# FFTAI/Wiki-GRx-Gym

Measured on AMD Instinct MI355X. Metric: env-steps/sec GR1T1 rough-terrain @4096 envs, higher is better.
Workload: dtype f32

## Files before the change

wiki-grx-gym_amd/csrc/grx_ppo.hip:

```cpp
#include <hip/hip_runtime.h>
#include <stdint.h>
#include "../../include/grx_ppo.h"

namespace {
constexpr int MAXA = 32;
constexpr int NTHR = 256;
constexpr int NRED = 3 + MAXA;

__device__ inline float nmax(float a, float b) { return (a > b || a != a) ? a : b; }
__device__ inline float nmin(float a, float b) { return (a < b || a != a) ? a : b; }

__device__ inline double wave_sum(double v) {
#pragma unroll
    for (int o = 32; o > 0; o >>= 1) v += __shfl_down(v, o);
    return v;
}

template <int A>
__global__ __launch_bounds__(NTHR) void ppo_loss_kernel(int B, const float* __restrict__ mu, const float* __restrict__ stdp,
                                                         const float* __restrict__ value, const float* __restrict__ actions,
                                                         const float* __restrict__ old_logp, const float* __restrict__ old_mu,
                                                         const float* __restrict__ old_sigma, const float* __restrict__ adv_,
                                                         const float* __restrict__ ret_, const float* __restrict__ tv_,
                                                         float clip, float vcoef, int use_clipped,
                                                         float* __restrict__ d_mu, float* __restrict__ d_value, double* __restrict__ partials) {
    const int i = blockIdx.x * NTHR + threadIdx.x;
    float red[3 + A];
#pragma unroll
    for (int k = 0; k < 3 + A; ++k) red[k] = 0.f;
    if (i < B) {
        const float invB = 1.0f / (float)B;
        float sg[A], df[A];
        float logp = 0.f, kl = 0.f;
#pragma unroll
        for (int k = 0; k < A; ++k) {
            const float s = stdp[k], m = mu[(size_t)i * A + k];
            sg[k] = s;
            df[k] = actions[(size_t)i * A + k] - m;
            logp += -(df[k] * df[k]) / (2.0f * s * s) - logf(s) - 0.9189385332046727f;
            const float os = old_sigma[(size_t)i * A + k], dm = old_mu[(size_t)i * A + k] - m;
            kl += logf(s / os + 1.e-5f) + (os * os + dm * dm) / (2.0f * s * s) - 0.5f;
        }
        const float adv = adv_[i];
        const float ratio = expf(logp - old_logp[i]);
        const float lo = 1.0f - clip, hi = 1.0f + clip;
        const float rc = nmin(nmax(ratio, lo), hi);
        const float s1 = -adv * ratio, s2 = -adv * rc;
        const float surr = nmax(s1, s2);
        const float w1 = s1 > s2 ? 1.f : (s1 == s2 ? 0.5f : 0.f), w2 = 1.f - w1;
        const float in_range = (ratio >= lo && ratio <= hi) ? 1.f : 0.f;
        const float g_ratio = -adv * (w1 + w2 * in_range);
        const float g_logp = g_ratio * ratio * invB;
#pragma unroll
        for (int k = 0; k < A; ++k) {
            const float s = sg[k], inv2 = 1.0f / (s * s);
            const float half = 0.5f * inv2;
            const float np = 0.f * (g_logp * (((df[k] * df[k] * half) * half) * 2.0f * (2.0f * s)) - g_logp / s);
            d_mu[(size_t)i * A + k] = g_logp * df[k] * inv2 + np;
            red[3 + k] = g_logp * (df[k] * df[k] * inv2 / s - 1.0f / s) + np;
        }
        const float v = value[i], ret = ret_[i];
        float vl, gv;
        if (use_clipped) {
            const float tv = tv_[i];
            const float dv = v - tv;
            const float vc = tv + nmin(nmax(dv, -clip), clip);
            const float l1 = (v - ret) * (v - ret), l2 = (vc - ret) * (vc - ret);
            vl = nmax(l1, l2);
            const float u1 = l1 > l2 ? 1.f : (l1 == l2 ? 0.5f : 0.f), u2 = 1.f - u1;
            const float vin = (dv >= -clip && dv <= clip) ? 1.f : 0.f;
            gv = u1 * 2.0f * (v - ret) + (vin != 0.f ? u2 * 2.0f * (vc - ret) : 0.f);
        } else {
            vl = (ret - v) * (ret - v);
            gv = -2.0f * (ret - v);
        }
        d_value[i] = vcoef * gv * invB;
        red[0] = surr; red[1] = vl; red[2] = kl;
    }
    __shared__ double s_red[NTHR / 64][3 + A];
    const int lane = threadIdx.x & 63, wv = threadIdx.x >> 6;
#pragma unroll
    for (int k = 0; k < 3 + A; ++k) {
        const double t = wave_sum((double)red[k]);
        if (lane == 0) s_red[wv][k] = t;
    }
    __syncthreads();
    if (threadIdx.x < 3 + A) {
        double t = 0.0;
#pragma unroll
        for (int w = 0; w < NTHR / 64; ++w) t += s_red[w][threadIdx.x];
        partials[(size_t)blockIdx.x * NRED + threadIdx.x] = t;
    }
}

__global__ __launch_bounds__(64) void ppo_loss_finalize(int B, int A, int nblk, const double* __restrict__ partials,
                                                         const float* __restrict__ stdp, float vcoef, float ecoef,
                                                         float* __restrict__ out, float* __restrict__ d_std) {
    const int k = threadIdx.x;
    double t = 0.0;
    constexpr int STAGE = 4096;
    __shared__ double s_p[STAGE];
    const bool staged = nblk * NRED <= STAGE;
    if (staged) {
        for (int i = k; i < nblk * NRED; i += 64) s_p[i] = partials[i];
        __syncthreads();
    }
    if (k < 3 + A)
        for (int b = 0; b < nblk; ++b) t += staged ? s_p[b * NRED + k] : partials[(size_t)b * NRED + k];
    __shared__ double s_t[64];
    s_t[k] = t;
    __syncthreads();
    if (k >= 3 && k < 3 + A) d_std[k - 3] = (float)t - ecoef / stdp[k - 3];
    if (k == 0) {
        const float surr = (float)(s_t[0] / (double)B), vl = (float)(s_t[1] / (double)B), klm = (float)(s_t[2] / (double)B);
        float ent = 0.f;
        for (int a = 0; a < A; ++a) ent += 1.4189385332046727f + logf(stdp[a]);
        out[0] = surr; out[1] = vl; out[2] = surr + vcoef * vl - ecoef * ent; out[3] = klm;
    }
}

template <int A>
void launch(int nblk, hipStream_t st, int B, const float* mu, const float* stdp, const float* value, const float* actions,
            const float* old_logp, const float* old_mu, const float* old_sigma, const float* adv, const float* ret, const float* tv,
            float clip, float vcoef, int use_clipped, float* d_mu, float* d_value, double* partials) {
    hipLaunchKernelGGL(ppo_loss_kernel<A>, dim3(nblk), dim3(NTHR), 0, st, B, mu, stdp, value, actions, old_logp, old_mu, old_sigma,
                       adv, ret, tv, clip, vcoef, use_clipped, d_mu, d_value, partials);
}

constexpr int CS_ROWS = 256;
__global__ __launch_bounds__(256) void colsum_partial(int rows, int cols, const float* __restrict__ x, float* __restrict__ partials) {
    const int lane = threadIdx.x & 63, wv = threadIdx.x >> 6;
    const int col = blockIdx.x * 64 + lane;
    const int r0 = blockIdx.y * CS_ROWS, r1 = min(rows, r0 + CS_ROWS);
    float acc = 0.f;
    if (col < cols) {
        float a0 = 0.f, a1 = 0.f, a2 = 0.f, a3 = 0.f;
        int r = r0 + wv;
        for (; r + 12 < r1; r += 16) {
            a0 += x[(size_t)r * cols + col]; a1 += x[(size_t)(r + 4) * cols + col];
            a2 += x[(size_t)(r + 8) * cols + col]; a3 += x[(size_t)(r + 12) * cols + col];
        }
// ... 403 lines not shown
```

wiki-grx-gym_amd/rl/fused_loss.py:

```python
import ctypes as C
import os

import torch

_LIB = None


def load_ppo_library():
    global _LIB
    if _LIB is None:
        path = os.environ.get("GRX_PPO_LIB") or os.path.join(os.path.dirname(os.path.dirname(os.path.abspath(__file__))), "csrc", "libgrx_ppo.so")
        if not os.path.exists(path):
            raise RuntimeError(f"{path} is missing: build it with `python -c 'import __graft_entry__ as g; g.build()'` "
                               "(there is no silent fallback for CUDA tensors; set GRX_PPO_FUSED_LOSS=0 to use the torch expression)")
        lib = C.CDLL(path)
        fp = C.c_void_p
        lib.grx_ppo_loss.restype = C.c_int
        lib.grx_ppo_loss.argtypes = [C.c_int, C.c_int] + [fp] * 10 + [C.c_float, C.c_float, C.c_float, C.c_int] + [fp] * 5 + [C.c_void_p]
        lib.grx_ppo_loss_partials_size.restype = C.c_int
        lib.grx_ppo_loss_partials_size.argtypes = [C.c_int]
        lib.grx_ppo_colsum.restype = C.c_int
        lib.grx_ppo_colsum.argtypes = [C.c_int, C.c_int, fp, fp, fp, C.c_void_p]
        lib.grx_ppo_colsum_partials_size.restype = C.c_int
        lib.grx_ppo_colsum_partials_size.argtypes = [C.c_int, C.c_int]
# ... 63 lines not shown
        lib.grx_est_forward.argtypes = [fp, C.c_int, C.c_int, fp, C.c_int, fp, C.POINTER(C.c_int), fp, fp, C.c_void_p]
        lib.grx_gae_partials_size.restype = C.c_int
        lib.grx_gae_partials_size.argtypes = [C.c_int, C.c_int]
        lib.grx_gae_returns.restype = C.c_int
        lib.grx_gae_returns.argtypes = [C.c_int, C.c_int] + [fp] * 4 + [C.c_float] * 3 + [fp] * 10 + [C.c_void_p]
        lib.grx_gp_seed.restype = C.c_int
        lib.grx_gp_seed.argtypes = [C.c_int, C.c_int] + [fp] * 4 + [C.c_void_p]
        lib.grx_gp_gate.restype = C.c_int
        lib.grx_gp_gate.argtypes = [C.c_int, C.c_int] + [fp] * 3 + [C.c_void_p]
        lib.grx_gp_sqnorm_partials_size.restype = C.c_int
        lib.grx_gp_sqnorm_partials_size.argtypes = [C.c_int, C.c_int]
        lib.grx_gp_sqnorm.restype = C.c_int
        lib.grx_gp_sqnorm.argtypes = [C.c_int, C.c_int] + [fp] * 3 + [C.c_void_p]
        lib.grx_gp_gate_backward.restype = C.c_int
        lib.grx_gp_gate_backward.argtypes = [C.c_int, C.c_int] + [fp] * 8 + [C.c_void_p]
        lib.grx_gp_seed_backward.restype = C.c_int
        lib.grx_gp_seed_backward.argtypes = [C.c_int, C.c_int] + [fp] * 8 + [C.c_void_p]
        lib.grx_ln_elu_forward.restype = C.c_int
        lib.grx_ln_elu_forward.argtypes = [C.c_int, C.c_int, fp, fp, fp, C.c_float, fp, fp, fp, C.c_void_p]
        lib.grx_ln_elu_backward_partials_size.restype = C.c_int
        lib.grx_ln_elu_backward_partials_size.argtypes = [C.c_int, C.c_int]
        lib.grx_ln_elu_backward.restype = C.c_int
        lib.grx_ln_elu_backward.argtypes = [C.c_int, C.c_int] + [fp] * 11 + [C.c_void_p]
        _LIB = lib
    return _LIB


TAIL_MAX = 24


class _TailTensors(C.Structure):
    _fields_ = [("n", C.c_int), ("pad", C.c_int), ("param", C.c_void_p * TAIL_MAX), ("grad", C.c_void_p * TAIL_MAX),
                ("exp_avg", C.c_void_p * TAIL_MAX), ("exp_avg_sq", C.c_void_p * TAIL_MAX), ("step", C.c_void_p * TAIL_MAX),
                ("numel", C.c_longlong * TAIL_MAX)]


class _TailArgs(C.Structure):
    _fields_ = [("loss", C.c_void_p), ("bad_flag", C.c_void_p), ("kl", C.c_void_p), ("lr", C.c_void_p), ("value_loss", C.c_void_p),
                ("surrogate_loss", C.c_void_p), ("sums", C.c_void_p), ("partials", C.c_void_p), ("adaptive", C.c_int), ("pad", C.c_int),
                ("desired_kl", C.c_float), ("lr_min", C.c_float), ("lr_max", C.c_float), ("max_grad_norm", C.c_float),
                ("beta1", C.c_double), ("beta2", C.c_double), ("eps", C.c_double)]


class StepTail:

    @staticmethod
# ... 113 lines not shown
        with torch.cuda.device(raw.device):
            rc = lib.grx_ppo_loss_sd(B, A, raw_c.data_ptr(), int(bool(log_std)), value_c.data_ptr(), *[t.data_ptr() for t in data],
                                     float(clip_param), float(value_loss_coef), float(entropy_coef), int(bool(use_clipped_value_loss)),
                                     out.data_ptr(), d_raw.data_ptr(), d_value.data_ptr(), partials.data_ptr(), C.c_void_p(stream))
        if rc != 0:
            raise RuntimeError(f"grx_ppo_loss_sd failed ({rc}): batch {B}, num_actions {A}")
        ctx.save_for_backward(d_raw, d_value)
        ctx.value_shape = value.shape
        return out

    @staticmethod
    def backward(ctx, g):
        d_raw, d_value = ctx.saved_tensors
        gl = g[2]
        return (d_raw * gl, (d_value * gl).reshape(ctx.value_shape)) + (None,) * 12


def fused_ppo_loss_sd(raw, value, actions, old_logp, old_mu, old_sigma, advantages, returns, target_values,
                      log_std, clip_param, value_loss_coef, entropy_coef, use_clipped_value_loss):
    return FusedPPOLossSD.apply(raw, value, actions, old_logp, old_mu, old_sigma, advantages, returns, target_values,
                                log_std, clip_param, value_loss_coef, entropy_coef, use_clipped_value_loss)


def colsum(x):
    lib = load_ppo_library()
    x = _f32c(x)
    rows, cols = x.shape
    out = torch.empty(cols, device=x.device, dtype=torch.float32)
    partials = torch.empty(lib.grx_ppo_colsum_partials_size(rows, cols), device=x.device, dtype=torch.float32)
    with torch.cuda.device(x.device):
        rc = lib.grx_ppo_colsum(rows, cols, x.data_ptr(), out.data_ptr(), partials.data_ptr(),
                                C.c_void_p(torch.cuda.current_stream(x.device).cuda_stream))
    if rc != 0:
        raise RuntimeError(f"grx_ppo_colsum failed ({rc}): {rows} x {cols}")
    return out


def elu_backward_colsum(dy, y):
    lib = load_ppo_library()
    dy, y = _f32c(dy), _f32c(y)
    rows, cols = dy.shape
    dz = torch.empty_like(dy)
    out = torch.empty(cols, device=dy.device, dtype=torch.float32)
    partials = torch.empty(lib.grx_ppo_colsum_partials_size(rows, cols), device=dy.device, dtype=torch.float32)
    with torch.cuda.device(dy.device):
        rc = lib.grx_ppo_elu_backward_colsum(rows, cols, dy.data_ptr(), y.data_ptr(), dz.data_ptr(), out.data_ptr(), partials.data_ptr(),
# ... 297 lines not shown
```

wiki-grx-gym_amd/rl/modules.py:

```python
import torch
import torch.nn as nn
from torch.distributions import Normal

PRECISIONS = ("fp32", "bf16")
_ACTIVATIONS = {"elu": nn.ELU, "selu": nn.SELU, "relu": nn.ReLU, "crelu": nn.ReLU, "lrelu": nn.LeakyReLU,
                "tanh": nn.Tanh, "sigmoid": nn.Sigmoid}


def get_activation(name):
    if name not in _ACTIVATIONS:
        print("invalid activation function!")
        return None
    return _ACTIVATIONS[name]()


import os

_FUSED_ELU_FORWARD = os.environ.get("GRX_PPO_FUSED_FWD", "1") != "0"
_FUSED_ELU_BACKWARD = os.environ.get("GRX_PPO_FUSED_ELU", "1") != "0"
_TRAIN_LINEAR = os.environ.get("GRX_PPO_LINEAR", "colsum")


class _TrainLinear(torch.autograd.Function):

# ... 139 lines not shown
        layers.append(nn.Linear(dims[-1], output_size))
        self.model = nn.Sequential(*layers)
        self.precision = "fp32"

    def set_precision(self, precision):
        if precision not in PRECISIONS:
            raise ValueError(f"precision must be one of {PRECISIONS}, not {precision!r}")
        if precision == "bf16":
            from .fused_loss import _linears_of
            if _linears_of(self) is None:
                raise ValueError("precision='bf16' needs an MLP of Linear -> ELU(alpha=1) hidden layers")
        self.precision = precision

    @torch.jit.unused
    def _forward_bf16(self, x):
        if not (x.is_cuda and x.dtype == torch.float32):
            raise RuntimeError("an MLP set to precision='bf16' runs on a HIP device with fp32 input only (there is no CPU path)")
        if torch.is_grad_enabled():
            return self._forward_train(x, bf16=True)
        from .fused_loss import mlp_forward
        return mlp_forward(self, x.reshape(-1, x.shape[-1])).reshape(*x.shape[:-1], self.output_size)

    @torch.jit.unused
    def _forward_train(self, x, bf16=False):
        mods = list(self.model)
        i = 0
        while i < len(mods):
            m = mods[i]
            if isinstance(m, nn.Linear) and i + 2 < len(mods) and isinstance(mods[i + 1], nn.LayerNorm) and isinstance(mods[i + 2], nn.ELU) \
                    and mods[i + 2].alpha == 1.0 and mods[i + 1].elementwise_affine and mods[i + 1].bias is not None:
                x = _TrainLinearLNELU.apply(x, m.weight, m.bias, mods[i + 1].weight, mods[i + 1].bias, mods[i + 1].eps)
                i += 3
                continue
            if isinstance(m, nn.Linear) and i + 1 < len(mods) and isinstance(mods[i + 1], nn.ELU) and mods[i + 1].alpha == 1.0 \
                    and (_FUSED_ELU_BACKWARD or bf16):
                x = _TrainLinearELU.apply(x, m.weight, m.bias, bf16)
                i += 2
                continue
            x = _TrainLinear.apply(x, m.weight, m.bias) if isinstance(m, nn.Linear) else m(x)
            i += 1
        return x

    def forward(self, x):
        if not torch.jit.is_scripting():
            if self.precision == "bf16":
                return self._forward_bf16(x)
            if x.is_cuda and torch.is_grad_enabled() and x.dtype == torch.float32 and _TRAIN_LINEAR == "colsum":
                return self._forward_train(x)
        return self.model(x)


NOISE_STD_TYPES = ("scalar", "log")


class MeanHead(nn.Module):

    def __init__(self, actor, num_actions: int):
        super().__init__()
        self.actor, self.num_actions = actor, int(num_actions)

    def forward(self, x):
        return torch.narrow(self.actor(x), -1, 0, self.num_actions)


# ... 136 lines not shown
```

wiki-grx-gym_amd/rl/ppo.py:

```python
import contextlib
import os

import torch
import torch.distributed as dist
from .fused_loss import fused_ppo_loss, fused_ppo_loss_sd, mlp_can_fuse, mlp_forward, policy_act
import torch.nn as nn
import torch.optim as optim

from .modules import PRECISIONS, ActorCriticMLP
from .storage import RolloutStorage


def _collective_path():
    return _world() > 1 or (os.environ.get("GRX_PPO_FORCE_BUCKET") == "1" and dist.is_available() and dist.is_initialized())


def _capture_mode():
    return "thread_local" if dist.is_available() and dist.is_initialized() else "global"


def _noise_std(ac):
    return ac.noise_std() if hasattr(ac, "noise_std") else ac.std


# ... 29 lines not shown
        if precision == "bf16" and torch.device(device).type != "cuda":
            raise ValueError(f"PPO: precision='bf16' runs on a HIP device only, not on {device!r} (there is no CPU path)")
        if precision != "fp32" and not hasattr(actor_critic, "set_precision"):
            raise ValueError(f"PPO: {type(actor_critic).__name__} has no set_precision(): precision={precision!r} is not available")
        self.precision = precision
        self.device = device
        self.desired_kl, self.schedule, self.mean_kl = desired_kl, schedule, 0.0
        self.learning_rate, self.learning_rate_min, self.learning_rate_max = learning_rate, learning_rate_min, learning_rate_max
        self.actor_critic = actor_critic.to(device)
        if precision == "bf16" and getattr(actor_critic, "layer_norm", False):
            raise ValueError("PPO: --layer_norm and --precision bf16 exclude each other: the bf16 products cover Linear -> ELU hidden layers only")
        if hasattr(self.actor_critic, "set_precision"):
            self.actor_critic.set_precision(precision)
        self.storage_class = storage_class
        self.storage, self.transition = None, None
        self._device_lr = torch.device(device).type == "cuda"
        self._use_graph = self._device_lr and os.environ.get("GRX_PPO_GRAPH", "1") not in ("0", "")
        if self._use_graph:
            from . import modules
            if modules._TRAIN_LINEAR != "colsum":
                print("PPO: GRX_PPO_LINEAR=" + modules._TRAIN_LINEAR + " -> the minibatch step runs eagerly (GRX_PPO_GRAPH=0)")
                self._use_graph = False
        self._fused_loss = self._device_lr and os.environ.get("GRX_PPO_FUSED_LOSS", "1") != "0"
        self._fused_store = self._device_lr and os.environ.get("GRX_PPO_FUSED_STORE", "1") != "0"
        self._fused_tail = self._device_lr and os.environ.get("GRX_PPO_FUSED_TAIL", "1") != "0"
        self._tail = None
        self._graph, self._graph_mb, self._static, self._sums, self._restore_opt = None, None, None, None, None
        self._use_act_graph = self._device_lr and os.environ.get("GRX_PPO_ACT_GRAPH", "1") not in ("0", "")
        self._act_graph, self._act_key, self._act_in, self._act_out = None, None, None, None
        self._two_streams = self._use_graph and os.environ.get("GRX_PPO_TWO_STREAMS", "1") != "0"
        self._aux_stream = None
        self._recurrent = bool(getattr(actor_critic, "is_recurrent", False))
        self._state_dependent = bool(getattr(actor_critic, "state_dependent_std", False))
        if self._state_dependent:
            if self._recurrent:
                raise ValueError("PPO: --state_dependent_std and --recurrent exclude each other: a recurrent policy with a state-dependent "
                                 "sigma is not implemented")
            if symmetry is not None:
                raise ValueError("PPO: --state_dependent_std and --symmetry exclude each other: a mirror map of the [mean | s] output is "
                                 "not implemented")
            if _world() > 1:
                raise NotImplementedError("PPO: --state_dependent_std with a world size above 1 is not implemented: it trains in one "
                                          "process only")
        if self._recurrent:
            if _world() > 1:
                raise NotImplementedError("PPO: a recurrent policy trains in one process only")
# ... 416 lines not shown
                bad = self._clip_found_inf(~torch.isfinite(loss.detach()))
                self.optimizer.step()
                with torch.no_grad():
                    sums[0] += torch.where(bad, 0.0, value_loss.detach())
                    sums[1] += torch.where(bad, 0.0, surrogate_loss.detach())
                    sums[2] = kl_mean
        host = sums.tolist()
        if self._device_lr:
            self.mean_kl = host[2]
            self.learning_rate = float(self._lr_t.item())
        return host[0] / self.num_updates, host[1] / self.num_updates

    @contextlib.contextmanager
    def _blas_for_update(self):
        prev_blas = torch.backends.cuda.preferred_blas_library()
        if os.environ.get("GRX_PPO_BLAS", "rocblas") == "rocblas":
            torch.backends.cuda.preferred_blas_library("cublas")
        try:
            yield
        finally:
            torch.backends.cuda.preferred_blas_library(prev_blas)

    def _losses(self, obs, cobs, actions, target_values, advantages, returns, old_logp, old_mu, old_sigma):
        mu, value = self._forward(obs, cobs)
        return self._loss_terms(mu, value, actions, target_values, advantages, returns, old_logp, old_mu, old_sigma)

    def _loss_is_fused(self):
        ac = self.actor_critic
        return self._fused_loss and not ac.fixed_std and ac.num_actor_output <= 32

    def _forward(self, obs, cobs, actor=None):
        ac = self.actor_critic
        if actor is not None:
            if not self._loss_is_fused():
                return actor(obs), ac.evaluate(cobs)
        elif self._state_dependent and not self._loss_is_fused():
            return ac.actor(obs), ac.evaluate(cobs)
        elif not self._loss_is_fused():
            ac.update_distribution(obs)
            return ac.action_mean, ac.evaluate(cobs)
        else:
            actor = ac.actor
        if self._two_streams and torch.backends.cuda.preferred_blas_library() == torch._C._BlasBackend.Cublas:
            cur = torch.cuda.current_stream(self.device)
            if self._aux_stream is None:
                self._aux_stream = torch.cuda.Stream(device=self.device)
            self._aux_stream.wait_stream(cur)
            with torch.cuda.stream(self._aux_stream):
# ... 567 lines not shown
```

wiki-grx-gym_amd/rl/runner.py:

```python
import json
import os
import random
import statistics
import time
from collections import deque

import torch
import torch.distributed as dist

from .distillation import Distillation, StudentTeacher, read_teacher
from .history import HistoryPolicy, ObsHistory
from .modules import ActorCriticMLP
from .normalizer import EmpiricalNormalization, NormalizedPolicy, normalize_step
from .ppo import PPO
from .recurrent import ActorCriticRecurrent, RecurrentPolicy
from .storage import RolloutStorage

_POLICIES = {"ActorCriticMLP": ActorCriticMLP, "ActorCritic": ActorCriticMLP, "ActorCriticRecurrent": ActorCriticRecurrent}
_ALGORITHMS = {"PPO": PPO, "Distillation": Distillation}


class _ScalarLog:

    def __init__(self, log_dir):
# ... 101 lines not shown
            self._alt_inputs = self._distill_inputs
        else:
            policy_in = actor_in + (len(estimator_cfg["cols"]) if estimator_cfg is not None else 0)
            actor_critic = policy_cls(policy_in, critic_in, env.num_actions, **self.policy_cfg).to(device)
            extra = {}
            if self.symmetry is not None:
                from .symmetry import build_maps
                self._symmetry_maps = extra["symmetry_maps"] = build_maps(env, device, self.obs_history_length, self.critic_obs_history_length,
                                                                           self.privileged_actor)
            self.algorithm = _ALGORITHMS[self.cfg["algorithm_class_name"]](actor_critic=actor_critic, device=device, **self.algorithm_cfg, **extra)
            if self.privileged_actor:
                self._alt_inputs = self._privileged_inputs
            if rnd_cfg is not None:
                from .rnd import RandomNetworkDistillation
                state = rnd_cfg.get("state", "privileged")
                self.rnd = self.algorithm.rnd = RandomNetworkDistillation(
                    env.num_pri_obs if state == "privileged" else env.num_obs, env.num_envs, self.cfg["num_steps_per_env"], device,
                    **rnd_cfg)
            if estimator_cfg is not None:
                from .estimator import StateEstimator
                self.estimator = StateEstimator(actor_in, env.num_obs, env.num_pri_obs, env.num_envs, self.cfg["num_steps_per_env"], device,
                                                targets=estimator_cfg["targets"], hidden_dims=estimator_cfg["hidden_dims"],
                                                learning_rate=estimator_cfg["learning_rate"], num_epochs=estimator_cfg["num_epochs"])
        self.alg = self.algorithm
        self.num_steps_per_env, self.save_interval = self.cfg["num_steps_per_env"], self.cfg["save_interval"]
        self.exact_resume = bool(self.cfg.get("exact_resume", False))
        if self.exact_resume and dist.is_available() and dist.is_initialized() and dist.get_world_size() > 1:
            raise NotImplementedError("exact_resume: one process only (with more ranks every rank holds its own env shard)")
        if self.exact_resume and self.distill_from is not None:
            raise NotImplementedError("exact_resume: not available for a distillation run (--distill_from)")
        self.empirical_normalization = bool(self.cfg.get("empirical_normalization", False))
        self.obs_normalizer = self.critic_obs_normalizer = None
        if self.empirical_normalization:
            if not self.privileged_actor:
                self.obs_normalizer = EmpiricalNormalization(actor_in).to(device)
            if env.num_pri_obs is not None and self.distill_from is None:
                self.critic_obs_normalizer = EmpiricalNormalization(critic_in).to(device)
        if self._symmetry_maps is not None and self.empirical_normalization:
            actor_norm = self.obs_normalizer if self.obs_normalizer is not None else self.critic_obs_normalizer
            self._symmetry_maps.obs_normalizer = actor_norm
            self._symmetry_maps.critic_obs_normalizer = self.critic_obs_normalizer if self.critic_obs_normalizer is not None else actor_norm
            self._symmetry_maps.refresh()
        self._pending_state = None
        self._log_buffers = None
        self._next_iteration = None
        self.algorithm.init_storage(env.num_envs, self.num_steps_per_env)
# ... 654 lines not shown
```

Before: 96.59 million.

## Fuse final actor/critic linear layers into the PPO loss kernel with custom backward

```diff
diff --git a/include/grx_ppo_head.h b/include/grx_ppo_head.h
--- /dev/null
+++ b/include/grx_ppo_head.h
@@ -0,0 +1,27 @@
+#ifndef GRX_PPO_HEAD_H
+#define GRX_PPO_HEAD_H
+#ifdef __cplusplus
+extern "C" {
+#endif
+
+#define GRX_HEAD_MAX_ACTIONS 32
+#define GRX_HEAD_MAX_HIDDEN 512
+
+int grx_head_workspace_size(int batch, int num_actions, int hidden);
+
+int grx_head_loss(int batch, int num_actions, int hidden, const float* h_a, const float* W_a, const float* b_a, const float* std,
+                  const float* h_c, const float* W_v, const float* b_v,
+                  const float* actions, const float* old_logp, const float* old_mu, const float* old_sigma,
+                  const float* advantages, const float* returns, const float* target_values,
+                  float clip_param, float value_loss_coef, float entropy_coef, int use_clipped_value_loss,
+                  float* mu, float* value, float* out, float* d_mu, float* d_std, float* d_value, float* loss_partials, void* stream);
+
+int grx_head_backward(int batch, int num_actions, int hidden, const float* d_mu, const float* d_value, const float* d_std, const float* gl,
+                      const float* h_a, const float* h_c, const float* W_a, const float* W_v,
+                      float* dH_a, float* dH_c, float* dW_a, float* db_a, float* dW_v, float* db_v, float* d_std_out,
+                      float* workspace, void* stream);
+
+#ifdef __cplusplus
+}
+#endif
+#endif
diff --git a/wiki-grx-gym_amd/csrc/grx_ppo.hip b/wiki-grx-gym_amd/csrc/grx_ppo.hip
--- a/wiki-grx-gym_amd/csrc/grx_ppo.hip
+++ b/wiki-grx-gym_amd/csrc/grx_ppo.hip
@@ -2,20 +2,9 @@
 #include <stdint.h>
 #include "../../include/grx_ppo.h"
 
+#include "grx_ppo_loss_row.h"
+
 namespace {
-constexpr int MAXA = 32;
-constexpr int NTHR = 256;
-constexpr int NRED = 3 + MAXA;
-
-__device__ inline float nmax(float a, float b) { return (a > b || a != a) ? a : b; }
-__device__ inline float nmin(float a, float b) { return (a < b || a != a) ? a : b; }
-
-__device__ inline double wave_sum(double v) {
-#pragma unroll
-    for (int o = 32; o > 0; o >>= 1) v += __shfl_down(v, o);
-    return v;
-}
-
 template <int A>
 __global__ __launch_bounds__(NTHR) void ppo_loss_kernel(int B, const float* __restrict__ mu, const float* __restrict__ stdp,
                                                          const float* __restrict__ value, const float* __restrict__ actions,
@@ -29,94 +18,13 @@
 #pragma unroll
     for (int k = 0; k < 3 + A; ++k) red[k] = 0.f;
     if (i < B) {
-        const float invB = 1.0f / (float)B;
-        float sg[A], df[A];
-        float logp = 0.f, kl = 0.f;
-#pragma unroll
-        for (int k = 0; k < A; ++k) {
-            const float s = stdp[k], m = mu[(size_t)i * A + k];
-            sg[k] = s;
-            df[k] = actions[(size_t)i * A + k] - m;
-            logp += -(df[k] * df[k]) / (2.0f * s * s) - logf(s) - 0.9189385332046727f;
-            const float os = old_sigma[(size_t)i * A + k], dm = old_mu[(size_t)i * A + k] - m;
-            kl += logf(s / os + 1.e-5f) + (os * os + dm * dm) / (2.0f * s * s) - 0.5f;
-        }
-        const float adv = adv_[i];
-        const float ratio = expf(logp - old_logp[i]);
-        const float lo = 1.0f - clip, hi = 1.0f + clip;
-        const float rc = nmin(nmax(ratio, lo), hi);
-        const float s1 = -adv * ratio, s2 = -adv * rc;
-        const float surr = nmax(s1, s2);
-        const float w1 = s1 > s2 ? 1.f : (s1 == s2 ? 0.5f : 0.f), w2 = 1.f - w1;
-        const float in_range = (ratio >= lo && ratio <= hi) ? 1.f : 0.f;
-        const float g_ratio = -adv * (w1 + w2 * in_range);
-        const float g_logp = g_ratio * ratio * invB;
-#pragma unroll
-        for (int k = 0; k < A; ++k) {
-            const float s = sg[k], inv2 = 1.0f / (s * s);
-            const float half = 0.5f * inv2;
-            const float np = 0.f * (g_logp * (((df[k] * df[k] * half) * half) * 2.0f * (2.0f * s)) - g_logp / s);
-            d_mu[(size_t)i * A + k] = g_logp * df[k] * inv2 + np;
-            red[3 + k] = g_logp * (df[k] * df[k] * inv2 / s - 1.0f / s) + np;
-        }
-        const float v = value[i], ret = ret_[i];
-        float vl, gv;
-        if (use_clipped) {
-            const float tv = tv_[i];
-            const float dv = v - tv;
-            const float vc = tv + nmin(nmax(dv, -clip), clip);
-            const float l1 = (v - ret) * (v - ret), l2 = (vc - ret) * (vc - ret);
-            vl = nmax(l1, l2);
-            const float u1 = l1 > l2 ? 1.f : (l1 == l2 ? 0.5f : 0.f), u2 = 1.f - u1;
-            const float vin = (dv >= -clip && dv <= clip) ? 1.f : 0.f;
-            gv = u1 * 2.0f * (v - ret) + (vin != 0.f ? u2 * 2.0f * (vc - ret) : 0.f);
-        } else {
-            vl = (ret - v) * (ret - v);
-            gv = -2.0f * (ret - v);
-        }
-        d_value[i] = vcoef * gv * invB;
-        red[0] = surr; red[1] = vl; red[2] = kl;
+        float m[A];
+#pragma unroll
+        for (int k = 0; k < A; ++k) m[k] = mu[(size_t)i * A + k];
+        ppo_loss_row<A>(i, B, m, value[i], stdp, actions, old_logp, old_mu, old_sigma, adv_, ret_, tv_, clip, vcoef, use_clipped, d_mu, d_value, red);
     }
     __shared__ double s_red[NTHR / 64][3 + A];
-    const int lane = threadIdx.x & 63, wv = threadIdx.x >> 6;
-#pragma unroll
-    for (int k = 0; k < 3 + A; ++k) {
-        const double t = wave_sum((double)red[k]);
-        if (lane == 0) s_red[wv][k] = t;
-    }
-    __syncthreads();
-    if (threadIdx.x < 3 + A) {
-        double t = 0.0;
-#pragma unroll
-        for (int w = 0; w < NTHR / 64; ++w) t += s_red[w][threadIdx.x];
-        partials[(size_t)blockIdx.x * NRED + threadIdx.x] = t;
-    }
-}
-
-__global__ __launch_bounds__(64) void ppo_loss_finalize(int B, int A, int nblk, const double* __restrict__ partials,
-                                                         const float* __restrict__ stdp, float vcoef, float ecoef,
-                                                         float* __restrict__ out, float* __restrict__ d_std) {
-    const int k = threadIdx.x;
-    double t = 0.0;
-    constexpr int STAGE = 4096;
-    __shared__ double s_p[STAGE];
-    const bool staged = nblk * NRED <= STAGE;
-    if (staged) {
-        for (int i = k; i < nblk * NRED; i += 64) s_p[i] = partials[i];
-        __syncthreads();
-    }
-    if (k < 3 + A)
-        for (int b = 0; b < nblk; ++b) t += staged ? s_p[b * NRED + k] : partials[(size_t)b * NRED + k];
-    __shared__ double s_t[64];
-    s_t[k] = t;
-    __syncthreads();
-    if (k >= 3 && k < 3 + A) d_std[k - 3] = (float)t - ecoef / stdp[k - 3];
-    if (k == 0) {
-        const float surr = (float)(s_t[0] / (double)B), vl = (float)(s_t[1] / (double)B), klm = (float)(s_t[2] / (double)B);
-        float ent = 0.f;
-        for (int a = 0; a < A; ++a) ent += 1.4189385332046727f + logf(stdp[a]);
-        out[0] = surr; out[1] = vl; out[2] = surr + vcoef * vl - ecoef * ent; out[3] = klm;
-    }
+    ppo_loss_block_sums<A>(red, s_red, partials);
 }
 
 template <int A>
diff --git a/wiki-grx-gym_amd/csrc/grx_ppo_head.hip b/wiki-grx-gym_amd/csrc/grx_ppo_head.hip
--- /dev/null
+++ b/wiki-grx-gym_amd/csrc/grx_ppo_head.hip
@@ -0,0 +1,235 @@
+#include <hip/hip_runtime.h>
+#include <stdint.h>
+#include "../../include/grx_ppo_head.h"
+#include "grx_ppo_loss_row.h"
+
+namespace {
+constexpr int MAXH = GRX_HEAD_MAX_HIDDEN;
+constexpr int HB_ROWS = 256;
+constexpr int HB_RB = 16;
+
+template <int A>
+__global__ __launch_bounds__(NTHR) void head_loss_kernel(int B, int H, const float* __restrict__ h_a, const float* __restrict__ W_a,
+                                                          const float* __restrict__ b_a, const float* __restrict__ stdp,
+                                                          const float* __restrict__ h_c, const float* __restrict__ W_v,
+                                                          const float* __restrict__ b_v, const float* __restrict__ actions,
+                                                          const float* __restrict__ old_logp, const float* __restrict__ old_mu,
+                                                          const float* __restrict__ old_sigma, const float* __restrict__ adv_,
+                                                          const float* __restrict__ ret_, const float* __restrict__ tv_,
+                                                          float clip, float vcoef, int use_clipped, float* __restrict__ mu,
+                                                          float* __restrict__ value, float* __restrict__ d_mu, float* __restrict__ d_value,
+                                                          double* __restrict__ partials) {
+    extern __shared__ double s_dyn[];
+    float* sW = reinterpret_cast<float*>(s_dyn);
+    for (int j = threadIdx.x; j < A * H; j += NTHR) sW[j] = W_a[j];
+    __syncthreads();
+    const int i = blockIdx.x * NTHR + threadIdx.x;
+    float red[3 + A];
+#pragma unroll
+    for (int k = 0; k < 3 + A; ++k) red[k] = 0.f;
+    if (i < B) {
+        float m[A];
+#pragma unroll
+        for (int a = 0; a < A; ++a) m[a] = 0.f;
+        float v = 0.f;
+        const float4* __restrict__ xa = reinterpret_cast<const float4*>(h_a + (size_t)i * H);
+        const float4* __restrict__ xc = reinterpret_cast<const float4*>(h_c + (size_t)i * H);
+#pragma unroll 2
+        for (int k4 = 0; k4 < H / 4; ++k4) {
+            const float4 x = xa[k4], c = xc[k4];
+#pragma unroll
+            for (int a = 0; a < A; ++a) {
+                const float4 w = *reinterpret_cast<const float4*>(sW + a * H + 4 * k4);
+                m[a] = fmaf(x.x, w.x, m[a]); m[a] = fmaf(x.y, w.y, m[a]); m[a] = fmaf(x.z, w.z, m[a]); m[a] = fmaf(x.w, w.w, m[a]);
+            }
+            v = fmaf(c.x, W_v[4 * k4], v); v = fmaf(c.y, W_v[4 * k4 + 1], v); v = fmaf(c.z, W_v[4 * k4 + 2], v); v = fmaf(c.w, W_v[4 * k4 + 3], v);
+        }
+#pragma unroll
+        for (int a = 0; a < A; ++a) {
+            m[a] += b_a[a];
+            mu[(size_t)i * A + a] = m[a];
+        }
+        v += b_v[0];
+        value[i] = v;
+        ppo_loss_row<A>(i, B, m, v, stdp, actions, old_logp, old_mu, old_sigma, adv_, ret_, tv_, clip, vcoef, use_clipped, d_mu, d_value, red);
+    }
+    __syncthreads();
+    ppo_loss_block_sums<A>(red, reinterpret_cast<double (*)[3 + A]>(s_dyn), partials);
+}
+
+template <int A>
+__device__ inline void head_backward_slab(const int B, const int H, const int cg, const float* __restrict__ d, const float* __restrict__ h,
+                                          const float* __restrict__ W, const double gl, float* __restrict__ dH, double* __restrict__ ws_dW,
+                                          double* __restrict__ ws_db, double* s_sum) {
+    const int lane = threadIdx.x & 63, wv = threadIdx.x >> 6;
+    const int col = cg * 64 + lane;
+    const int r0 = blockIdx.y * HB_ROWS, nrows = min(B - r0, HB_ROWS);
+    double* s_d = s_sum;
+    for (int j = threadIdx.x; j < nrows * A; j += 256) s_d[j] = (double)d[(size_t)r0 * A + j];
+    __syncthreads();
+    double w[A], acc[A];
+#pragma unroll
+    for (int a = 0; a < A; ++a) { acc[a] = 0.0; w[a] = col < H ? (double)W[(size_t)a * H + col] : 0.0; }
+    if (col < H) {
+        for (int rb = wv; rb < nrows; rb += 4 * HB_RB) {
+            float xs[HB_RB];
+#pragma unroll
+            for (int j = 0; j < HB_RB; ++j) xs[j] = h[(size_t)(r0 + min(rb + 4 * j, nrows - 1)) * H + col];
+#pragma unroll
+            for (int j = 0; j < HB_RB; ++j) {
+                const int r = rb + 4 * j;
+                if (r < nrows) {
+                    const double x = (double)xs[j];
+                    double g = 0.0;
+#pragma unroll
+                    for (int a = 0; a < A; ++a) {
+                        const double dv = s_d[r * A + a];
+                        g = fma(dv, w[a], g);
+                        acc[a] = fma(dv, x, acc[a]);
+                    }
+                    dH[(size_t)(r0 + r) * H + col] = (float)(gl * g);
+                }
+            }
+        }
+    }
+    double db = 0.0;
+    if (cg == 0 && lane < A)
+        for (int r = wv; r < nrows; r += 4) db += s_d[r * A + lane];
+    __syncthreads();
+    if (wv > 0) {
+#pragma unroll
+        for (int a = 0; a < A; ++a) s_sum[((wv - 1) * (A + 1) + a) * 64 + lane] = acc[a];
+        s_sum[((wv - 1) * (A + 1) + A) * 64 + lane] = db;
+    }
+    __syncthreads();
+    if (wv == 0) {
+        auto four = [&](const double own, const int a) {
+            return (own + s_sum[a * 64 + lane]) + (s_sum[((A + 1) + a) * 64 + lane] + s_sum[(2 * (A + 1) + a) * 64 + lane]);
+        };
+        if (col < H) {
+#pragma unroll
+            for (int a = 0; a < A; ++a) ws_dW[(size_t)a * H + col] = four(acc[a], a);
+        }
+        if (cg == 0 && lane < A) ws_db[lane] = four(db, A);
+    }
+}
+
+template <int A>
+constexpr int head_backward_lds() {
+    return (HB_ROWS * A > 3 * (A + 1) * 64) ? HB_ROWS * A : 3 * (A + 1) * 64;
+}
+
+template <int A>
+__global__ __launch_bounds__(256) void head_backward_kernel(int B, int H, const float* __restrict__ d_mu, const float* __restrict__ d_value,
+                                                             const float* __restrict__ glp, const float* __restrict__ h_a,
+                                                             const float* __restrict__ h_c, const float* __restrict__ W_a,
+                                                             const float* __restrict__ W_v, float* __restrict__ dH_a, float* __restrict__ dH_c,
+                                                             double* __restrict__ workspace) {
+    __shared__ double s_sum[head_backward_lds<A>()];
+    const int ncg = (H + 63) / 64;
+    const double gl = (double)glp[0];
+    double* ws = workspace + (size_t)blockIdx.y * ((size_t)A * H + A + H + 1);
+    if ((int)blockIdx.x < ncg)
+        head_backward_slab<A>(B, H, blockIdx.x, d_mu, h_a, W_a, gl, dH_a, ws, ws + (size_t)A * H, s_sum);
+    else
+        head_backward_slab<1>(B, H, blockIdx.x - ncg, d_value, h_c, W_v, gl, dH_c, ws + (size_t)A * H + A, ws + (size_t)A * H + A + H, s_sum);
+}
+
+__global__ __launch_bounds__(256) void head_backward_final(int A, int H, int nslab, const double* __restrict__ workspace, const float* __restrict__ glp,
+                                                            const float* __restrict__ d_std, float* __restrict__ dW_a, float* __restrict__ db_a,
+                                                            float* __restrict__ dW_v, float* __restrict__ db_v, float* __restrict__ d_std_out) {
+    const int S = A * H + A + H + 1;
+    const int j = blockIdx.x * 256 + threadIdx.x;
+    if (j >= S) {
+        if (j < S + A) d_std_out[j - S] = glp[0] * d_std[j - S];
+        return;
+    }
+    double t = 0.0;
+    int s = 0;
+    for (; s + 4 <= nslab; s += 4) {
+        const double p0 = workspace[(size_t)s * S + j], p1 = workspace[(size_t)(s + 1) * S + j];
+        const double p2 = workspace[(size_t)(s + 2) * S + j], p3 = workspace[(size_t)(s + 3) * S + j];
+        t += p0; t += p1; t += p2; t += p3;
+    }
+    for (; s < nslab; ++s) t += workspace[(size_t)s * S + j];
+    const float o = (float)(t * (double)glp[0]);
+    if (j < A * H) dW_a[j] = o;
+    else if (j < A * H + A) db_a[j - A * H] = o;
+    else if (j < A * H + A + H) dW_v[j - A * H - A] = o;
+    else db_v[0] = o;
+}
+
+bool sizes_ok(int B, int A, int H) {
+    return B >= 1 && B <= 65535 * HB_ROWS && A >= 1 && A <= MAXA && H >= 4 && H <= MAXH && H % 4 == 0;
+}
+
+template <int A>
+void launch_loss(int nblk, hipStream_t st, int B, int H, const float* h_a, const float* W_a, const float* b_a, const float* stdp, const float* h_c,
+                 const float* W_v, const float* b_v, const float* actions, const float* old_logp, const float* old_mu, const float* old_sigma,
+                 const float* adv, const float* ret, const float* tv, float clip, float vcoef, int use_clipped, float* mu, float* value,
+                 float* d_mu, float* d_value, double* partials) {
+    const size_t w_bytes = (size_t)A * H * sizeof(float), red_bytes = (size_t)(NTHR / 64) * (3 + A) * sizeof(double);
+    hipLaunchKernelGGL(head_loss_kernel<A>, dim3(nblk), dim3(NTHR), w_bytes > red_bytes ? w_bytes : red_bytes, st, B, H, h_a, W_a, b_a, stdp, h_c,
+                       W_v, b_v, actions, old_logp, old_mu, old_sigma, adv, ret, tv, clip, vcoef, use_clipped, mu, value, d_mu, d_value, partials);
+}
+
+template <int A>
+void launch_backward(int nslab, hipStream_t st, int B, int H, const float* d_mu, const float* d_value, const float* gl, const float* h_a,
+                     const float* h_c, const float* W_a, const float* W_v, float* dH_a, float* dH_c, double* workspace) {
+    hipLaunchKernelGGL(head_backward_kernel<A>, dim3(2 * ((H + 63) / 64), nslab), dim3(256), 0, st, B, H, d_mu, d_value, gl, h_a, h_c, W_a, W_v,
+                       dH_a, dH_c, workspace);
+}
+}
+
+#define GRX_HEAD_CASES                                                                                                                       \
+    GRX_HEAD_CASE(1) GRX_HEAD_CASE(2) GRX_HEAD_CASE(3) GRX_HEAD_CASE(4) GRX_HEAD_CASE(5) GRX_HEAD_CASE(6) GRX_HEAD_CASE(7) GRX_HEAD_CASE(8)  \
+    GRX_HEAD_CASE(9) GRX_HEAD_CASE(10) GRX_HEAD_CASE(11) GRX_HEAD_CASE(12) GRX_HEAD_CASE(13) GRX_HEAD_CASE(14) GRX_HEAD_CASE(15)             \
+    GRX_HEAD_CASE(16) GRX_HEAD_CASE(17) GRX_HEAD_CASE(18) GRX_HEAD_CASE(19) GRX_HEAD_CASE(20) GRX_HEAD_CASE(21) GRX_HEAD_CASE(22)            \
+    GRX_HEAD_CASE(23) GRX_HEAD_CASE(24) GRX_HEAD_CASE(25) GRX_HEAD_CASE(26) GRX_HEAD_CASE(27) GRX_HEAD_CASE(28) GRX_HEAD_CASE(29)            \
+    GRX_HEAD_CASE(30) GRX_HEAD_CASE(31) GRX_HEAD_CASE(32)
+
+extern "C" int grx_head_workspace_size(int batch, int num_actions, int hidden) {
+    if (!sizes_ok(batch, num_actions, hidden)) return 0;
+    const long long n = 2LL * ((batch + HB_ROWS - 1) / HB_ROWS) * ((long long)num_actions * hidden + num_actions + hidden + 1);
+    return n > 0x7fffffffLL ? 0 : (int)n;
+}
+
+extern "C" int grx_head_loss(int batch, int num_actions, int hidden, const float* h_a, const float* W_a, const float* b_a, const float* std,
+                             const float* h_c, const float* W_v, const float* b_v,
+                             const float* actions, const float* old_logp, const float* old_mu, const float* old_sigma,
+                             const float* advantages, const float* returns, const float* target_values,
+                             float clip_param, float value_loss_coef, float entropy_coef, int use_clipped_value_loss,
+                             float* mu, float* value, float* out, float* d_mu, float* d_std, float* d_value, float* loss_partials, void* stream) {
+    if (!sizes_ok(batch, num_actions, hidden)) return -1;
+    if (!h_a || !W_a || !b_a || !std || !h_c || !W_v || !b_v || !actions || !old_logp || !old_mu || !old_sigma || !advantages || !returns
+        || !target_values || !mu || !value || !out || !d_mu || !d_std || !d_value || !loss_partials) return -1;
+    if (((uintptr_t)h_a & 15) || ((uintptr_t)h_c & 15) || ((uintptr_t)loss_partials & 7)) return -1;
+    hipStream_t st = (hipStream_t)stream;
+    const int nblk = (batch + NTHR - 1) / NTHR;
+#define GRX_HEAD_CASE(A) case A: launch_loss<A>(nblk, st, batch, hidden, h_a, W_a, b_a, std, h_c, W_v, b_v, actions, old_logp, old_mu, old_sigma,   \
+                                                advantages, returns, target_values, clip_param, value_loss_coef, use_clipped_value_loss, mu, value, \
+                                                d_mu, d_value, (double*)loss_partials); break;
+    switch (num_actions) { GRX_HEAD_CASES }
+#undef GRX_HEAD_CASE
+    hipLaunchKernelGGL(ppo_loss_finalize, dim3(1), dim3(64), 0, st, batch, num_actions, nblk, (const double*)loss_partials, std, value_loss_coef,
+                       entropy_coef, out, d_std);
+    return hipGetLastError() == hipSuccess ? 0 : -2;
+}
+
+extern "C" int grx_head_backward(int batch, int num_actions, int hidden, const float* d_mu, const float* d_value, const float* d_std, const float* gl,
+                                 const float* h_a, const float* h_c, const float* W_a, const float* W_v,
+                                 float* dH_a, float* dH_c, float* dW_a, float* db_a, float* dW_v, float* db_v, float* d_std_out,
+                                 float* workspace, void* stream) {
+    if (!sizes_ok(batch, num_actions, hidden) || grx_head_workspace_size(batch, num_actions, hidden) == 0) return -1;
+    if (!d_mu || !d_value || !d_std || !gl || !h_a || !h_c || !W_a || !W_v || !dH_a || !dH_c || !dW_a || !db_a || !dW_v || !db_v || !d_std_out
+        || !workspace || ((uintptr_t)workspace & 7)) return -1;
+    hipStream_t st = (hipStream_t)stream;
+    const int nslab = (batch + HB_ROWS - 1) / HB_ROWS;
+#define GRX_HEAD_CASE(A) case A: launch_backward<A>(nslab, st, batch, hidden, d_mu, d_value, gl, h_a, h_c, W_a, W_v, dH_a, dH_c, (double*)workspace); break;
+    switch (num_actions) { GRX_HEAD_CASES }
+#undef GRX_HEAD_CASE
+    const int S = num_actions * hidden + num_actions + hidden + 1;
+    hipLaunchKernelGGL(head_backward_final, dim3((S + num_actions + 255) / 256), dim3(256), 0, st, num_actions, hidden, nslab, (const double*)workspace, gl, d_std,
+                       dW_a, db_a, dW_v, db_v, d_std_out);
+    return hipGetLastError() == hipSuccess ? 0 : -2;
+}
diff --git a/wiki-grx-gym_amd/csrc/grx_ppo_loss_row.h b/wiki-grx-gym_amd/csrc/grx_ppo_loss_row.h
--- /dev/null
+++ b/wiki-grx-gym_amd/csrc/grx_ppo_loss_row.h
@@ -0,0 +1,118 @@
+#ifndef GRX_PPO_LOSS_ROW_H
+#define GRX_PPO_LOSS_ROW_H
+#include <hip/hip_runtime.h>
+
+namespace {
+constexpr int MAXA = 32;
+constexpr int NTHR = 256;
+constexpr int NRED = 3 + MAXA;
+
+__device__ inline float nmax(float a, float b) { return (a > b || a != a) ? a : b; }
+__device__ inline float nmin(float a, float b) { return (a < b || a != a) ? a : b; }
+
+__device__ inline double wave_sum(double v) {
+#pragma unroll
+    for (int o = 32; o > 0; o >>= 1) v += __shfl_down(v, o);
+    return v;
+}
+
+template <int A>
+__device__ inline void ppo_loss_row(const int i, const int B, const float (&mu_i)[A], const float v, const float* __restrict__ stdp,
+                                    const float* __restrict__ actions, const float* __restrict__ old_logp,
+                                    const float* __restrict__ old_mu, const float* __restrict__ old_sigma,
+                                    const float* __restrict__ adv_, const float* __restrict__ ret_, const float* __restrict__ tv_,
+                                    const float clip, const float vcoef, const int use_clipped,
+                                    float* __restrict__ d_mu, float* __restrict__ d_value, float (&red)[3 + A]) {
+    const float invB = 1.0f / (float)B;
+    float sg[A], df[A];
+    float logp = 0.f, kl = 0.f;
+#pragma unroll
+    for (int k = 0; k < A; ++k) {
+        const float s = stdp[k], m = mu_i[k];
+        sg[k] = s;
+        df[k] = actions[(size_t)i * A + k] - m;
+        logp += -(df[k] * df[k]) / (2.0f * s * s) - logf(s) - 0.9189385332046727f;
+        const float os = old_sigma[(size_t)i * A + k], dm = old_mu[(size_t)i * A + k] - m;
+        kl += logf(s / os + 1.e-5f) + (os * os + dm * dm) / (2.0f * s * s) - 0.5f;
+    }
+    const float adv = adv_[i];
+    const float ratio = expf(logp - old_logp[i]);
+    const float lo = 1.0f - clip, hi = 1.0f + clip;
+    const float rc = nmin(nmax(ratio, lo), hi);
+    const float s1 = -adv * ratio, s2 = -adv * rc;
+    const float surr = nmax(s1, s2);
+    const float w1 = s1 > s2 ? 1.f : (s1 == s2 ? 0.5f : 0.f), w2 = 1.f - w1;
+    const float in_range = (ratio >= lo && ratio <= hi) ? 1.f : 0.f;
+    const float g_ratio = -adv * (w1 + w2 * in_range);
+    const float g_logp = g_ratio * ratio * invB;
+#pragma unroll
+    for (int k = 0; k < A; ++k) {
+        const float s = sg[k], inv2 = 1.0f / (s * s);
+        const float half = 0.5f * inv2;
+        const float np = 0.f * (g_logp * (((df[k] * df[k] * half) * half) * 2.0f * (2.0f * s)) - g_logp / s);
+        d_mu[(size_t)i * A + k] = g_logp * df[k] * inv2 + np;
+        red[3 + k] = g_logp * (df[k] * df[k] * inv2 / s - 1.0f / s) + np;
+    }
+    const float ret = ret_[i];
+    float vl, gv;
+    if (use_clipped) {
+        const float tv = tv_[i];
+        const float dv = v - tv;
+        const float vc = tv + nmin(nmax(dv, -clip), clip);
+        const float l1 = (v - ret) * (v - ret), l2 = (vc - ret) * (vc - ret);
+        vl = nmax(l1, l2);
+        const float u1 = l1 > l2 ? 1.f : (l1 == l2 ? 0.5f : 0.f), u2 = 1.f - u1;
+        const float vin = (dv >= -clip && dv <= clip) ? 1.f : 0.f;
+        gv = u1 * 2.0f * (v - ret) + (vin != 0.f ? u2 * 2.0f * (vc - ret) : 0.f);
+    } else {
+        vl = (ret - v) * (ret - v);
+        gv = -2.0f * (ret - v);
+    }
+    d_value[i] = vcoef * gv * invB;
+    red[0] = surr; red[1] = vl; red[2] = kl;
+}
+
+template <int A>
+__device__ inline void ppo_loss_block_sums(const float (&red)[3 + A], double (*s_red)[3 + A], double* __restrict__ partials) {
+    const int lane = threadIdx.x & 63, wv = threadIdx.x >> 6;
+#pragma unroll
+    for (int k = 0; k < 3 + A; ++k) {
+        const double t = wave_sum((double)red[k]);
+        if (lane == 0) s_red[wv][k] = t;
+    }
+    __syncthreads();
+    if (threadIdx.x < 3 + A) {
+        double t = 0.0;
+#pragma unroll
+        for (int w = 0; w < NTHR / 64; ++w) t += s_red[w][threadIdx.x];
+        partials[(size_t)blockIdx.x * NRED + threadIdx.x] = t;
+    }
+}
+
+__global__ __launch_bounds__(64) void ppo_loss_finalize(int B, int A, int nblk, const double* __restrict__ partials,
+                                                         const float* __restrict__ stdp, float vcoef, float ecoef,
+                                                         float* __restrict__ out, float* __restrict__ d_std) {
+    const int k = threadIdx.x;
+    double t = 0.0;
+    constexpr int STAGE = 4096;
+    __shared__ double s_p[STAGE];
+    const bool staged = nblk * NRED <= STAGE;
+    if (staged) {
+        for (int i = k; i < nblk * NRED; i += 64) s_p[i] = partials[i];
+        __syncthreads();
+    }
+    if (k < 3 + A)
+        for (int b = 0; b < nblk; ++b) t += staged ? s_p[b * NRED + k] : partials[(size_t)b * NRED + k];
+    __shared__ double s_t[64];
+    s_t[k] = t;
+    __syncthreads();
+    if (k >= 3 && k < 3 + A) d_std[k - 3] = (float)t - ecoef / stdp[k - 3];
+    if (k == 0) {
+        const float surr = (float)(s_t[0] / (double)B), vl = (float)(s_t[1] / (double)B), klm = (float)(s_t[2] / (double)B);
+        float ent = 0.f;
+        for (int a = 0; a < A; ++a) ent += 1.4189385332046727f + logf(stdp[a]);
+        out[0] = surr; out[1] = vl; out[2] = surr + vcoef * vl - ecoef * ent; out[3] = klm;
+    }
+}
+}
+#endif
diff --git a/wiki-grx-gym_amd/rl/fused_loss.py b/wiki-grx-gym_amd/rl/fused_loss.py
--- a/wiki-grx-gym_amd/rl/fused_loss.py
+++ b/wiki-grx-gym_amd/rl/fused_loss.py
@@ -109,6 +109,12 @@
         lib.grx_ln_elu_backward_partials_size.argtypes = [C.c_int, C.c_int]
         lib.grx_ln_elu_backward.restype = C.c_int
         lib.grx_ln_elu_backward.argtypes = [C.c_int, C.c_int] + [fp] * 11 + [C.c_void_p]
+        lib.grx_head_workspace_size.restype = C.c_int
+        lib.grx_head_workspace_size.argtypes = [C.c_int] * 3
+        lib.grx_head_loss.restype = C.c_int
+        lib.grx_head_loss.argtypes = [C.c_int] * 3 + [fp] * 14 + [C.c_float, C.c_float, C.c_float, C.c_int] + [fp] * 7 + [C.c_void_p]
+        lib.grx_head_backward.restype = C.c_int
+        lib.grx_head_backward.argtypes = [C.c_int] * 3 + [fp] * 16 + [C.c_void_p]
         _LIB = lib
     return _LIB
 
@@ -268,6 +274,77 @@
                                 log_std, clip_param, value_loss_coef, entropy_coef, use_clipped_value_loss)
 
 
+HEAD_MAX_ACTIONS, HEAD_MAX_HIDDEN = 32, 512
+
+
+def head_shapes_supported(A, H):
+    return 1 <= A <= HEAD_MAX_ACTIONS and 4 <= H <= HEAD_MAX_HIDDEN and H % 4 == 0
+
+
+def head_loss_forward(h_a, W_a, b_a, std, h_c, W_v, b_v, actions, old_logp, old_mu, old_sigma, advantages, returns, target_values,
+                      clip_param, value_loss_coef, entropy_coef, use_clipped_value_loss):
+    lib = load_ppo_library()
+    (B, H), A = h_a.shape, W_a.shape[0]
+    dev = h_a.device
+    out = torch.empty(4, device=dev, dtype=torch.float32)
+    mu, d_mu = (torch.empty(B, A, device=dev, dtype=torch.float32) for _ in range(2))
+    value, d_value = (torch.empty(B, device=dev, dtype=torch.float32) for _ in range(2))
+    d_std = torch.empty(A, device=dev, dtype=torch.float32)
+    partials = torch.empty(max(1, lib.grx_ppo_loss_partials_size(B)), device=dev, dtype=torch.float32)
+    ins = (h_a, W_a, b_a, std, h_c, W_v, b_v, actions, old_logp, old_mu, old_sigma, advantages, returns, target_values)
+    with torch.cuda.device(dev):
+        rc = lib.grx_head_loss(B, A, H, *[t.data_ptr() for t in ins], float(clip_param), float(value_loss_coef), float(entropy_coef),
+                               int(bool(use_clipped_value_loss)), mu.data_ptr(), value.data_ptr(), out.data_ptr(), d_mu.data_ptr(),
+                               d_std.data_ptr(), d_value.data_ptr(), partials.data_ptr(), C.c_void_p(torch.cuda.current_stream(dev).cuda_stream))
+    if rc != 0:
+        raise RuntimeError(f"grx_head_loss failed ({rc}): batch {B}, num_actions {A}, hidden {H}")
+    return out, mu, value, d_mu, d_std, d_value
+
+
+def head_loss_backward(d_mu, d_value, d_std, gl, h_a, h_c, W_a, W_v):
+    lib = load_ppo_library()
+    (B, H), A = h_a.shape, W_a.shape[0]
+    dev = h_a.device
+    dH_a, dH_c = (torch.empty(B, H, device=dev, dtype=torch.float32) for _ in range(2))
+    dW_a, db_a, d_std_out = torch.empty_like(W_a), torch.empty(A, device=dev, dtype=torch.float32), torch.empty_like(d_std)
+    dW_v, db_v = torch.empty(1, H, device=dev, dtype=torch.float32), torch.empty(1, device=dev, dtype=torch.float32)
+    ws = torch.empty(max(1, lib.grx_head_workspace_size(B, A, H)), device=dev, dtype=torch.float32)
+    with torch.cuda.device(dev):
+        rc = lib.grx_head_backward(B, A, H, d_mu.data_ptr(), d_value.data_ptr(), d_std.data_ptr(), gl.data_ptr(), h_a.data_ptr(), h_c.data_ptr(),
+                                   W_a.data_ptr(), W_v.data_ptr(), dH_a.data_ptr(), dH_c.data_ptr(), dW_a.data_ptr(), db_a.data_ptr(),
+                                   dW_v.data_ptr(), db_v.data_ptr(), d_std_out.data_ptr(), ws.data_ptr(),
+                                   C.c_void_p(torch.cuda.current_stream(dev).cuda_stream))
+    if rc != 0:
+        raise RuntimeError(f"grx_head_backward failed ({rc}): batch {B}, num_actions {A}, hidden {H}")
+    return dH_a, dH_c, dW_a, db_a, dW_v, db_v, d_std_out
+
+
+class FusedHeadLoss(torch.autograd.Function):
+
+    @staticmethod
+    def forward(ctx, h_a, W_a, b_a, std, h_c, W_v, b_v, actions, old_logp, old_mu, old_sigma, advantages, returns, target_values,
+                clip_param, value_loss_coef, entropy_coef, use_clipped_value_loss):
+        h_a, W_a, b_a, std, h_c, W_v, b_v = (_f32c(t) for t in (h_a, W_a, b_a, std, h_c, W_v, b_v))
+        data = [_f32c(t) for t in (actions, old_logp, old_mu, old_sigma, advantages, returns, target_values)]
+        out, _, _, d_mu, d_std, d_value = head_loss_forward(h_a, W_a, b_a, std, h_c, W_v, b_v, *data, clip_param, value_loss_coef,
+                                                            entropy_coef, use_clipped_value_loss)
+        ctx.save_for_backward(h_a, h_c, W_a, W_v, d_mu, d_std, d_value)
+        return out
+
+    @staticmethod
+    def backward(ctx, g):
+        h_a, h_c, W_a, W_v, d_mu, d_std, d_value = ctx.saved_tensors
+        gl = _f32c(g)[2:3]
+        dH_a, dH_c, dW_a, db_a, dW_v, db_v, d_std_g = head_loss_backward(d_mu, d_value, d_std, gl, h_a, h_c, W_a, W_v)
+        return (dH_a, dW_a, db_a, d_std_g, dH_c, dW_v, db_v) + (None,) * 11
+
+
+def fused_head_loss(h_a, W_a, b_a, std, h_c, W_v, b_v, actions, old_logp, old_mu, old_sigma, advantages, returns, target_values,
+                    clip_param, value_loss_coef, entropy_coef, use_clipped_value_loss):
+    return FusedHeadLoss.apply(h_a, W_a, b_a, std, h_c, W_v, b_v, actions, old_logp, old_mu, old_sigma, advantages, returns, target_values,
+                               clip_param, value_loss_coef, entropy_coef, use_clipped_value_loss)
+
+
 def colsum(x):
     lib = load_ppo_library()
     x = _f32c(x)
diff --git a/wiki-grx-gym_amd/rl/modules.py b/wiki-grx-gym_amd/rl/modules.py
--- a/wiki-grx-gym_amd/rl/modules.py
+++ b/wiki-grx-gym_amd/rl/modules.py
@@ -185,8 +185,8 @@
         return mlp_forward(self, x.reshape(-1, x.shape[-1])).reshape(*x.shape[:-1], self.output_size)
 
     @torch.jit.unused
-    def _forward_train(self, x, bf16=False):
-        mods = list(self.model)
+    def _forward_train(self, x, bf16=False, trunk=False):
+        mods = list(self.model)[:-1] if trunk else list(self.model)
         i = 0
         while i < len(mods):
             m = mods[i]
@@ -203,6 +203,10 @@
             x = _TrainLinear.apply(x, m.weight, m.bias) if isinstance(m, nn.Linear) else m(x)
             i += 1
         return x
+
+    @torch.jit.unused
+    def forward_trunk(self, x):
+        return self._forward_train(x, bf16=self.precision == "bf16", trunk=True)
 
     def forward(self, x):
         if not torch.jit.is_scripting():
diff --git a/wiki-grx-gym_amd/rl/ppo.py b/wiki-grx-gym_amd/rl/ppo.py
--- a/wiki-grx-gym_amd/rl/ppo.py
+++ b/wiki-grx-gym_amd/rl/ppo.py
@@ -75,6 +75,8 @@
                 print("PPO: GRX_PPO_LINEAR=" + modules._TRAIN_LINEAR + " -> the minibatch step runs eagerly (GRX_PPO_GRAPH=0)")
                 self._use_graph = False
         self._fused_loss = self._device_lr and os.environ.get("GRX_PPO_FUSED_LOSS", "1") != "0"
+        self._fused_head = self._device_lr and os.environ.get("GRX_PPO_FUSED_HEAD", "1") != "0"
+        self.head_fused = None
         self._fused_store = self._device_lr and os.environ.get("GRX_PPO_FUSED_STORE", "1") != "0"
         self._fused_tail = self._device_lr and os.environ.get("GRX_PPO_FUSED_TAIL", "1") != "0"
         self._tail = None
@@ -537,8 +539,52 @@
             torch.backends.cuda.preferred_blas_library(prev_blas)
 
     def _losses(self, obs, cobs, actions, target_values, advantages, returns, old_logp, old_mu, old_sigma):
+        self.head_fused = self._head_is_fused(obs, cobs)
+        if self.head_fused:
+            return self._losses_head(obs, cobs, actions, target_values, advantages, returns, old_logp, old_mu, old_sigma)
         mu, value = self._forward(obs, cobs)
         return self._loss_terms(mu, value, actions, target_values, advantages, returns, old_logp, old_mu, old_sigma)
+
+    def _head_is_fused(self, obs, cobs):
+        from .fused_loss import head_shapes_supported
+        from . import modules
+        ac = self.actor_critic
+        if not (self._fused_head and self._loss_is_fused()) or self._state_dependent or self._recurrent or self._layer_norm \
+                or self.precision != "fp32" or self.value_norm is not None or self.symmetry is not None or self.smooth is not None \
+                or self.grad_penalty_coef is not None or self.rnd is not None or modules._TRAIN_LINEAR != "colsum":
+            return False
+        actor, critic = getattr(ac, "actor", None), getattr(ac, "critic", None)
+        if type(actor) is not modules.MLP or type(critic) is not modules.MLP or len(actor.model) < 2 or len(critic.model) < 2:
+            return False
+        la, lc = actor.model[-1], critic.model[-1]
+        if not (isinstance(la, nn.Linear) and isinstance(lc, nn.Linear) and la.bias is not None and lc.bias is not None):
+            return False
+        return (lc.out_features == 1 and la.out_features == ac.num_actor_output and la.in_features == lc.in_features
+                and head_shapes_supported(la.out_features, la.in_features)
+                and all(x.is_cuda and x.dtype == torch.float32 and x.dim() == 2 for x in (obs, cobs)))
+
+    def _losses_head(self, obs, cobs, actions, target_values, advantages, returns, old_logp, old_mu, old_sigma):
+        from .fused_loss import fused_head_loss
+        ac = self.actor_critic
+        if self._two_streams and torch.backends.cuda.preferred_blas_library() == torch._C._BlasBackend.Cublas:
+            cur = torch.cuda.current_stream(self.device)
+            if self._aux_stream is None:
+                self._aux_stream = torch.cuda.Stream(device=self.device)
+            self._aux_stream.wait_stream(cur)
+            with torch.cuda.stream(self._aux_stream):
+                h_c = ac.critic.forward_trunk(cobs)
+            h_a = ac.actor.forward_trunk(obs)
+            cur.wait_stream(self._aux_stream)
+            h_c.record_stream(cur)
+        else:
+            h_a, h_c = ac.actor.forward_trunk(obs), ac.critic.forward_trunk(cobs)
+        la, lc = ac.actor.model[-1], ac.critic.model[-1]
+        out = fused_head_loss(h_a, la.weight, la.bias, _noise_std(ac), h_c, lc.weight, lc.bias, actions, old_logp, old_mu, old_sigma,
+                              advantages, returns, target_values, self.clip_param, self.value_loss_coef, self.entropy_coef,
+                              self.use_clipped_value_loss)
+        adaptive = self.desired_kl is not None and self.schedule == "adaptive"
+        kl_mean = out[3].detach() if adaptive else torch.zeros((), device=self.device)
+        return out[0], out[1], out[2], kl_mean
 
     def _loss_is_fused(self):
         ac = self.actor_critic
diff --git a/wiki-grx-gym_amd/rl/runner.py b/wiki-grx-gym_amd/rl/runner.py
--- a/wiki-grx-gym_amd/rl/runner.py
+++ b/wiki-grx-gym_amd/rl/runner.py
@@ -147,6 +147,8 @@
                 self.estimator = StateEstimator(actor_in, env.num_obs, env.num_pri_obs, env.num_envs, self.cfg["num_steps_per_env"], device,
                                                 targets=estimator_cfg["targets"], hidden_dims=estimator_cfg["hidden_dims"],
                                                 learning_rate=estimator_cfg["learning_rate"], num_epochs=estimator_cfg["num_epochs"])
+                if hasattr(self.algorithm, "_fused_head"):
+                    self.algorithm._fused_head = False
         self.alg = self.algorithm
         self.num_steps_per_env, self.save_interval = self.cfg["num_steps_per_env"], self.cfg["save_interval"]
         self.exact_resume = bool(self.cfg.get("exact_resume", False))
```

Result: no change. 96.72 million, median of 2 (+0.1%).
